# TtesseractT/Synthetic-Audio-Detection

Hardware: AMD Instinct MI355X
Metric: 4s@32kHz segments/sec end-to-end (mel+ResNet+ensemble), 1/2/4/8 MI355X (higher is better)
Workload: dtype bf16; 1 GPU; end-to-end inference: B int16 4 s segments resident in HBM -> mel front end -> ResNet-18@512x512 -> 6 binary heads -> merge (+RCCL all-gather of logits); heads=6, distinct_backbones=1, micro_batch=2048, parallelism=dp1, frontend_overlapped=True

## Files before the change

synthetic-audio-detection_amd/csrc/conv.hip:

```cpp
#include "common.hpp"
#include "kernels.hpp"
#include "igemm.hpp"

namespace sad {

template <int WM, int WN, int S>
constexpr int conv_smem_bytes() {
  constexpr int BM = 64 * WM, BN = 64 * WN;
  constexpr int main_b = S * (BM + BN) * 128;
  constexpr int epi_b = BM * (BN + 4) * 4;
  return main_b > epi_b ? main_b : epi_b;
}

template <typename T, int WM, int WN, int S>
__global__ __launch_bounds__(64 * WM * WN, 1) void conv_igemm_kernel(ConvArgs a) {
  static_assert(S == 2 || S == 3, "ring depth");
  constexpr int NW = WM * WN;
  constexpr int NT = 64 * NW;
  constexpr int BM = 64 * WM, BN = 64 * WN;
  constexpr int ES = sizeof(T);
  if (blockIdx.y > 0) {
    const int g = blockIdx.y;
    a.in = (const T*)a.in + g * a.in_gstride;
    a.wt = (const T*)a.wt + g * a.wt_gstride;
    a.bias = a.bias + g * a.bias_gstride;
    a.out = (T*)a.out + g * a.out_gstride;
  }
  constexpr int STAGE = (BM + BN) * 128;
  constexpr int QA = BM / 8 / NW;
  constexpr int QB = BN / 8 / NW;
  static_assert(QA * 8 * NW == BM && QB * 8 * NW == BN, "tile/wave mismatch");
  extern __shared__ __attribute__((aligned(16))) char smem[];

  const int tid = threadIdx.x, lane = tid & 63;
  const int wave = __builtin_amdgcn_readfirstlane(tid >> 6);
  const int wm = wave / WN, wn = wave % WN;
  const int n_tn = a.Cout / BN;
  const int wg = xcd_remap(blockIdx.x, gridDim.x);
  const int tn = wg % n_tn, tm = wg / n_tn;
  const int64_t m0 = (int64_t)tm * BM;
  const int n0 = tn * BN;
  const int HoWo = a.Ho * a.Wo;

  const __amdgpu_buffer_rsrc_t rin =
      __builtin_amdgcn_make_buffer_rsrc((void*)a.in, (short)0, (int)a.in_bytes, 0x00020000);
  const __amdgpu_buffer_rsrc_t rwt =
      __builtin_amdgcn_make_buffer_rsrc((void*)a.wt, (short)0, (int)a.wt_bytes, 0x00020000);
  const int pstride_b = (int)a.in_pstride * ES;

  const int lrow = lane >> 3;
  int aoff[QA], aiy[QA], aix[QA];
#pragma unroll
  for (int i = 0; i < QA; ++i) {
    const int r = 8 * (wave + NW * i) + lrow;
    const int c = (lane & 7) ^ ((r >> 1) & 7);
    const int64_t m = m0 + r;
    if (m < a.M) {
      const int b = (int)(m / HoWo);
      const int rem = (int)(m - (int64_t)b * HoWo);
      const int oy = rem / a.Wo, ox = rem - oy * a.Wo;
      aiy[i] = oy * a.stride - a.pad;
      aix[i] = ox * a.stride - a.pad;
      aoff[i] = ((b * a.H + aiy[i]) * a.W + aix[i]) * pstride_b + c * 16;
    } else {
      aiy[i] = -0x4000;
      aix[i] = -0x4000;
      aoff[i] = 0;
    }
  }
  const int ktot_b = a.KH * a.KW * a.Cin * ES;
  int boff[QB];
#pragma unroll
  for (int i = 0; i < QB; ++i) {
    const int r = 8 * (wave + NW * i) + lrow;
    const int c = (lane & 7) ^ (((r + BM) >> 1) & 7);
    boff[i] = (n0 + r) * ktot_b + c * 16;
  }
  const int cpt = a.Cin / (128 / ES);
  const int nk = a.KH * a.KW * cpt;

  const unsigned lds0 = (unsigned)(uintptr_t)(__attribute__((address_space(3))) char*)smem;
  auto issue = [&](int ks, int st) __attribute__((always_inline)) {
    const int tap = ks / cpt;
    const int ci0 = ks - tap * cpt;
    const int ky = tap / a.KW, kx = tap - ky * a.KW;
    const int toff = (ky * a.W + kx) * pstride_b + ci0 * 128;
    const unsigned sb = lds0 + st * STAGE;
#pragma unroll
    for (int i = 0; i < QA; ++i) {
      const int iy = aiy[i] + ky, ix = aix[i] + kx;
      const bool ok = ((unsigned)iy < (unsigned)a.H) && ((unsigned)ix < (unsigned)a.W);
      dma16(rin, ok ? aoff[i] + toff : 0x7FFFFFF0, sb + (wave + NW * i) * 1024);
    }
#pragma unroll
    for (int i = 0; i < QB; ++i) dma16(rwt, boff[i] + ks * 128, sb + BM * 128 + (wave + NW * i) * 1024);
  };

  f32x4 acc[4][4];
#pragma unroll
  for (int i = 0; i < 4; ++i)
#pragma unroll
    for (int j = 0; j < 4; ++j) acc[i][j] = f32x4{0.f, 0.f, 0.f, 0.f};

  const int fr = lane & 15, fg = lane >> 4;
  issue(0, 0);
  if (S == 3 && nk > 1) issue(1, 1);
  int st = 0;
  for (int ks = 0; ks < nk; ++ks) {
    if (S == 3 && ks + 1 < nk)
      asm volatile("s_waitcnt vmcnt(%0)" ::"n"(QA + QB) : "memory");
    else
      asm volatile("s_waitcnt vmcnt(0)" ::: "memory");
    __builtin_amdgcn_s_barrier();
    __builtin_amdgcn_sched_barrier(0);
    if (ks + S - 1 < nk) issue(ks + S - 1, S == 3 ? (st == 0 ? 2 : st - 1) : (st ^ 1));
    const char* base = smem + st * STAGE;
#pragma unroll
    for (int s = 0; s < 2; ++s) {
      uint4 af[4], bfr[4];
      const int c = fg + 4 * s;
#pragma unroll
      for (int i = 0; i < 4; ++i) {
        const int r = wm * 64 + i * 16 + fr;
        af[i] = *(const uint4*)(base + r * 128 + (swz(r, c) << 4));
      }
#pragma unroll
      for (int j = 0; j < 4; ++j) {
        const int r = BM + wn * 64 + j * 16 + fr;
        bfr[j] = *(const uint4*)(base + r * 128 + (swz(r, c) << 4));
      }
#pragma unroll
      for (int i = 0; i < 4; ++i)
#pragma unroll
        for (int j = 0; j < 4; ++j) mfma_chunk<T>(af[i], bfr[j], acc[i][j]);
    }
    st = st + 1 == S ? 0 : st + 1;
  }
  __syncthreads();

  float* ep = (float*)smem;
  constexpr int LDE = BN + 4;
#pragma unroll
  for (int i = 0; i < 4; ++i)
#pragma unroll
    for (int j = 0; j < 4; ++j)
#pragma unroll
      for (int r = 0; r < 4; ++r)
        ep[(wm * 64 + i * 16 + fg * 4 + r) * LDE + wn * 64 + j * 16 + fr] = acc[i][j][r];
  __syncthreads();
  constexpr int TPR = BN / 8;
  constexpr int RPP = NT / TPR;
  const int c8 = (tid % TPR) * 8;
  const float4 bias0 = *(const float4*)(a.bias + n0 + c8);
  const float4 bias1 = *(const float4*)(a.bias + n0 + c8 + 4);
  const T* __restrict__ res = (const T*)a.res;
  T* __restrict__ out = (T*)a.out;
  for (int row = tid / TPR; row < BM; row += RPP) {
    const int64_t m = m0 + row;
    if (m >= a.M) break;
    const float4 v0 = *(const float4*)(ep + row * LDE + c8);
    const float4 v1 = *(const float4*)(ep + row * LDE + c8 + 4);
    float v[8] = {v0.x + bias0.x, v0.y + bias0.y, v0.z + bias0.z, v0.w + bias0.w,
                  v1.x + bias1.x, v1.y + bias1.y, v1.z + bias1.z, v1.w + bias1.w};
    if (res) {
      const T* rp = res + m * a.res_pstride + n0 + c8;
      if constexpr (sizeof(T) == 2) {
        const uint4 q = *(const uint4*)rp;
        const u16* h = (const u16*)&q;
#pragma unroll
        for (int e = 0; e < 8; ++e) v[e] += bf2f(h[e]);
      } else {
        const float4 q0 = *(const float4*)rp, q1 = *(const float4*)(rp + 4);
        v[0] += q0.x; v[1] += q0.y; v[2] += q0.z; v[3] += q0.w;
        v[4] += q1.x; v[5] += q1.y; v[6] += q1.z; v[7] += q1.w;
      }
    }
    if (a.relu) {
#pragma unroll
      for (int e = 0; e < 8; ++e) v[e] = fmaxf(v[e], 0.f);
    }
    T* op = out + m * a.out_pstride + n0 + c8;
    if constexpr (sizeof(T) == 2) {
      uint4 q;
      u16* h = (u16*)&q;
#pragma unroll
      for (int e = 0; e < 8; ++e) h[e] = f2bf(v[e]);
      *(uint4*)op = q;
    } else {
      *(float4*)op = make_float4(v[0], v[1], v[2], v[3]);
      *(float4*)(op + 4) = make_float4(v[4], v[5], v[6], v[7]);
    }
  }
}

__device__ __forceinline__ float bilinear512(const float* __restrict__ map, int mh, int mw, float sh, float sw,
                                            int iy, int ix) {
  float fy = sh * (iy + 0.5f) - 0.5f;
  fy = fy < 0.f ? 0.f : fy;
  float fx = sw * (ix + 0.5f) - 0.5f;
  fx = fx < 0.f ? 0.f : fx;
  const int y0 = min((int)floorf(fy), mh - 1), x0 = min((int)floorf(fx), mw - 1);
  const int y1 = min(y0 + 1, mh - 1), x1 = min(x0 + 1, mw - 1);
  const float ly = fminf(fmaxf(fy - y0, 0.f), 1.f), lx = fminf(fmaxf(fx - x0, 0.f), 1.f);
  return (1.f - ly) * ((1.f - lx) * map[y0 * mw + x0] + lx * map[y0 * mw + x1]) +
         ly * ((1.f - lx) * map[y1 * mw + x0] + lx * map[y1 * mw + x1]);
}

constexpr int STEM_IMG_ROWS = 11;
constexpr int STEM_IMG_PITCH = 520;

template <typename T>
__global__ __launch_bounds__(256) void stem_kernel(StemArgs a) {
  constexpr int WPITCH = (64 * sizeof(T) + 16) / sizeof(T);
  __shared__ __attribute__((aligned(16))) float s_img[STEM_IMG_ROWS * STEM_IMG_PITCH];
  __shared__ __attribute__((aligned(16))) T s_w[64 * WPITCH];
  __shared__ __attribute__((aligned(16))) T s_pool[256 * 64];

  const int tid = threadIdx.x, lane = tid & 63, wave = tid >> 6;
  const int py = blockIdx.x;
  const int64_t b = blockIdx.y;
  const float* __restrict__ map = a.img ? nullptr : a.map + b * a.mh * a.mw;

  for (int i = tid; i < 64 * 64; i += 256) s_w[(i >> 6) * WPITCH + (i & 63)] = ((const T*)a.w)[i];
  const float sh = (float)a.mh / 512.f, sw = (float)a.mw / 512.f;
  for (int i = tid; i < STEM_IMG_ROWS * 517; i += 256) {
    const int tr = i / 517, tc = i - tr * 517;
    const int iy = 4 * py - 5 + tr, ix = tc - 3;
    float v = 0.f;
    if ((unsigned)iy < 512u && (unsigned)ix < 512u) {
      v = a.img ? a.img[(b * 512 + iy) * 512 + ix] : bilinear512(map, a.mh, a.mw, sh, sw, iy, ix);
      if constexpr (sizeof(T) == 2) v = bf2f(f2bf(v));
    }
    s_img[tr * STEM_IMG_PITCH + tc] = v;
  }
  __syncthreads();

  const int fr = lane & 15, fg = lane >> 4;
  int toff[16];
#pragma unroll
  for (int t = 0; t < 16; ++t) {
    int k;
    if constexpr (sizeof(T) == 2)
      k = 32 * (t >> 3) + 8 * fg + (t & 7);
    else
      k = 4 * t + fg;
    toff[t] = k < 49 ? (k / 7) * STEM_IMG_PITCH + (k % 7) : -1;
  }
  uint4 bw[4][2];
#pragma unroll
  for (int j = 0; j < 4; ++j) {
    const T* wr = s_w + (j * 16 + fr) * WPITCH;
    if constexpr (sizeof(T) == 2) {
      bw[j][0] = *(const uint4*)(wr + 8 * fg);
      bw[j][1] = *(const uint4*)(wr + 32 + 8 * fg);
    } else {
      bw[j][0] = *(const uint4*)(wr + 16 * fg);
      bw[j][1] = *(const uint4*)(wr + 16 * fg + 4);
    }
  }
  uint4 bw2[4][2];
  if constexpr (sizeof(T) == 4) {
#pragma unroll
    for (int j = 0; j < 4; ++j) {
      const T* wr = s_w + (j * 16 + fr) * WPITCH;
      bw2[j][0] = *(const uint4*)(wr + 16 * fg + 8);
      bw2[j][1] = *(const uint4*)(wr + 16 * fg + 12);
    }
  }

  f32x4 vmax[4][4];
#pragma unroll
  for (int i = 0; i < 4; ++i)
#pragma unroll
    for (int j = 0; j < 4; ++j) vmax[i][j] = f32x4{0.f, 0.f, 0.f, 0.f};

  for (int d = -1; d <= 1; ++d) {
    const int cr = 2 * py + d;
    if (cr < 0 || cr >= 256) continue;
    f32x4 acc[4][4];
#pragma unroll
    for (int i = 0; i < 4; ++i)
#pragma unroll
      for (int j = 0; j < 4; ++j) acc[i][j] = f32x4{0.f, 0.f, 0.f, 0.f};
#pragma unroll
    for (int i = 0; i < 4; ++i) {
      const int cx = wave * 64 + i * 16 + fr;
      const float* ib = s_img + (2 * d + 2) * STEM_IMG_PITCH + 2 * cx;
      float av[16];
#pragma unroll
      for (int t = 0; t < 16; ++t) av[t] = toff[t] >= 0 ? ib[toff[t]] : 0.f;
      if constexpr (sizeof(T) == 2) {
        uint4 a0, a1;
        u16* h0 = (u16*)&a0;
        u16* h1 = (u16*)&a1;
#pragma unroll
        for (int t = 0; t < 8; ++t) {
          h0[t] = f2bf(av[t]);
          h1[t] = f2bf(av[8 + t]);
        }
#pragma unroll
        for (int j = 0; j < 4; ++j) {
          mfma_chunk<u16>(a0, bw[j][0], acc[i][j]);
          mfma_chunk<u16>(a1, bw[j][1], acc[i][j]);
        }
      } else {
        const uint4 a0 = make_uint4(__float_as_uint(av[0]), __float_as_uint(av[1]), __float_as_uint(av[2]), __float_as_uint(av[3]));
        const uint4 a1 = make_uint4(__float_as_uint(av[4]), __float_as_uint(av[5]), __float_as_uint(av[6]), __float_as_uint(av[7]));
        const uint4 a2 = make_uint4(__float_as_uint(av[8]), __float_as_uint(av[9]), __float_as_uint(av[10]), __float_as_uint(av[11]));
        const uint4 a3 = make_uint4(__float_as_uint(av[12]), __float_as_uint(av[13]), __float_as_uint(av[14]), __float_as_uint(av[15]));
#pragma unroll
        for (int j = 0; j < 4; ++j) {
          mfma_chunk<float>(a0, bw[j][0], acc[i][j]);
          mfma_chunk<float>(a1, bw[j][1], acc[i][j]);
          mfma_chunk<float>(a2, bw2[j][0], acc[i][j]);
          mfma_chunk<float>(a3, bw2[j][1], acc[i][j]);
        }
      }
    }
#pragma unroll
    for (int j = 0; j < 4; ++j) {
      const float bj = a.bias[j * 16 + fr];
#pragma unroll
      for (int i = 0; i < 4; ++i)
#pragma unroll
        for (int r = 0; r < 4; ++r) {
          float v = fmaxf(acc[i][j][r] + bj, 0.f);
          if constexpr (sizeof(T) == 2) v = bf2f(f2bf(v));
          vmax[i][j][r] = fmaxf(vmax[i][j][r], v);
        }
    }
  }
#pragma unroll
  for (int i = 0; i < 4; ++i)
#pragma unroll
    for (int j = 0; j < 4; ++j)
#pragma unroll
      for (int r = 0; r < 4; ++r) {
        const int px = wave * 64 + i * 16 + fg * 4 + r;
        const float v = vmax[i][j][r];
        if constexpr (sizeof(T) == 2)
          s_pool[px * 64 + j * 16 + fr] = f2bf(v);
        else
          s_pool[px * 64 + j * 16 + fr] = v;
      }
  __syncthreads();
  T* __restrict__ out = (T*)a.out + ((b * 128 + py) * 128) * 64;
  for (int it = tid; it < 128 * 8; it += 256) {
    const int q = it >> 3, c0 = (it & 7) * 8;
    float m[8];
#pragma unroll
    for (int e = 0; e < 8; ++e) m[e] = 0.f;
    for (int px = 2 * q - 1; px <= 2 * q + 1; ++px) {
      if (px < 0 || px >= 256) continue;
#pragma unroll
      for (int e = 0; e < 8; ++e) {
        float v;
        if constexpr (sizeof(T) == 2)
          v = bf2f(s_pool[px * 64 + c0 + e]);
        else
          v = s_pool[px * 64 + c0 + e];
        m[e] = fmaxf(m[e], v);
      }
    }
    if constexpr (sizeof(T) == 2) {
      uint4 qv;
      u16* h = (u16*)&qv;
#pragma unroll
      for (int e = 0; e < 8; ++e) h[e] = f2bf(m[e]);
      *(uint4*)(out + q * 64 + c0) = qv;
    } else {
      *(float4*)(out + q * 64 + c0) = make_float4(m[0], m[1], m[2], m[3]);
      *(float4*)(out + q * 64 + c0 + 4) = make_float4(m[4], m[5], m[6], m[7]);
    }
  }
}

constexpr int STEM_P = 8;
constexpr int STEM_BAND_ROWS = 4 * STEM_P + 8;
constexpr int STEM_BPITCH = 544;
constexpr int STEM_HROWS = 12;
constexpr int STEM_UPITCH = 520;
constexpr int STEM_OPITCH = 128;
constexpr int STEM_WPITCH = 80;
__device__ __forceinline__ int stem_oswz(int q) { return ((q & 1) << 2) | (q & 2); }

typedef __bf16 stem_bf2 __attribute__((ext_vector_type(2)));
typedef float stem_f2 __attribute__((ext_vector_type(2)));
__device__ __forceinline__ uint32_t stem_pk(float lo, float hi) {
  return __builtin_bit_cast(uint32_t, __builtin_convertvector((stem_f2){lo, hi}, stem_bf2));
}
__device__ __forceinline__ uint32_t stem_relu2(uint32_t x) {
  uint32_t r;
  asm("v_pk_max_i16 %0, %1, 0" : "=v"(r) : "v"(x));
  return r;
}
template <int CTRL>
__device__ __forceinline__ float dppf(float v) {
  return __int_as_float(__builtin_amdgcn_update_dpp(0, __float_as_int(v), CTRL, 0xF, 0xF, true));
}

constexpr int STEM_OPITCH_X3 = 288;
constexpr int stem_u_build_floats() { return (STEM_HROWS + 1) * STEM_UPITCH + 4 * STEM_BAND_ROWS; }
template <bool X3>
constexpr int stem_u_floats() {
  return (X3 ? 128 * STEM_OPITCH_X3 / 4 : 128 * STEM_OPITCH / 4) + 256 > stem_u_build_floats()
             ? (X3 ? 128 * STEM_OPITCH_X3 / 4 : 128 * STEM_OPITCH / 4) + 256
             : stem_u_build_floats();
}

template <bool X3, bool TRAIN = false, bool X4 = false>
__global__ __launch_bounds__(256, X3 ? 1 : 2) void stem_bf16_kernel(StemArgs a) {
  static_assert(!(X3 && TRAIN), "the training stem is bf16");
  static_assert(!X4 || X3, "X4: the split stem's fourth product");
  constexpr int OPITCH = X3 ? STEM_OPITCH_X3 : STEM_OPITCH;
  __shared__ __attribute__((aligned(16))) u16 s_img[STEM_BAND_ROWS * STEM_BPITCH];
  __shared__ __attribute__((aligned(16))) u16 s_imgl[X3 ? STEM_BAND_ROWS * STEM_BPITCH : 8];
  __shared__ __attribute__((aligned(16))) u16 s_w[64 * STEM_WPITCH];
  __shared__ __attribute__((aligned(16))) u16 s_wl[X3 ? 64 * STEM_WPITCH : 8];
  __shared__ __attribute__((aligned(16))) float s_bias[64];
  __shared__ __attribute__((aligned(16))) float s_u[stem_u_floats<X3>()];
  char* s_out = (char*)s_u;
  float* s_edge = s_u + 128 * OPITCH / 4;

  const int tid = threadIdx.x, lane = tid & 63, wave = tid >> 6;
  const int py0 = blockIdx.x * STEM_P;
  const int64_t b = blockIdx.y;
  for (int i = tid; i < 64 * 8; i += 256) {
    const int co = i >> 3, c8 = (i & 7) * 8;
    uint4 wv = *(const uint4*)((const u16*)a.w + co * 64 + c8);
    if (TRAIN && a.bias[co] < 0.f) wv ^= make_uint4(0x80008000u, 0x80008000u, 0x80008000u, 0x80008000u);
    *(uint4*)(s_w + co * STEM_WPITCH + c8) = wv;
    if constexpr (X3)
      *(uint4*)(s_wl + co * STEM_WPITCH + c8) = *(const uint4*)((const u16*)a.w + 64 * 64 + co * 64 + c8);
  }
  auto put = [&](int i, float v) __attribute__((always_inline)) {
    const u16 h = f2bf(v);
    s_img[i] = h;
    if constexpr (X3) s_imgl[i] = f2bf(v - bf2f(h));
  };
  if (tid < 64) s_bias[tid] = TRAIN ? (a.bias[tid] < 0.f ? -1.f : 1.f) : a.bias[tid];
  constexpr int NBR = STEM_BAND_ROWS;
  if (TRAIN) {
    for (int i = tid; i < NBR * STEM_BPITCH; i += 256) {
      const int tr = i / STEM_BPITCH, tc = i - tr * STEM_BPITCH;
      const int iy = 4 * py0 - 5 + tr, ix = tc - 3;
      u16 v = 0;
      if ((unsigned)iy < 512u && (unsigned)ix < 512u) v = a.img16[(b * 512 + iy) * 512 + ix];
      s_img[i] = v;
    }
  } else if (a.img) {
    for (int i = tid; i < NBR * STEM_BPITCH; i += 256) {
      const int tr = i / STEM_BPITCH, tc = i - tr * STEM_BPITCH;
      const int iy = 4 * py0 - 5 + tr, ix = tc - 3;
      float v = 0.f;
      if ((unsigned)iy < 512u && (unsigned)ix < 512u) v = a.img[(b * 512 + iy) * 512 + ix];
      put(i, v);
    }
  } else {
    const float* __restrict__ map = a.map + b * a.mh * a.mw;
    const float sh = (float)a.mh / 512.f, sw = (float)a.mw / 512.f;
    auto src_row = [&](int iy, int& y0, int& y1, float& ly) {
      float fy = sh * (iy + 0.5f) - 0.5f;
      fy = fy < 0.f ? 0.f : fy;
      y0 = min((int)floorf(fy), a.mh - 1);
      y1 = min(y0 + 1, a.mh - 1);
      ly = fminf(fmaxf(fy - y0, 0.f), 1.f);
    };
    const int iy_lo = max(4 * py0 - 5, 0), iy_hi = min(4 * py0 - 5 + NBR - 1, 511);
    int ylo, yhi, t0, t1;
    float tl;
    src_row(iy_lo, ylo, t0, tl);
    src_row(iy_hi, t1, yhi, tl);
    const int nh = yhi - ylo + 1;
    if (nh <= STEM_HROWS) {
      constexpr int UP = STEM_UPITCH;
      float* s_zero = s_u + STEM_HROWS * UP;
      int4* s_rt = (int4*)(s_u + (STEM_HROWS + 1) * UP);
      int x0[2], x1[2];
      float lx[2];
#pragma unroll
      for (int c = 0; c < 2; ++c) {
        const int ix = tid + 256 * c;
        float fx = sw * (ix + 0.5f) - 0.5f;
        fx = fx < 0.f ? 0.f : fx;
        x0[c] = min((int)floorf(fx), a.mw - 1);
        x1[c] = min(x0[c] + 1, a.mw - 1);
        lx[c] = fminf(fmaxf(fx - x0[c], 0.f), 1.f);
      }
      float g0[STEM_HROWS][2], g1[STEM_HROWS][2];
#pragma unroll
      for (int r = 0; r < STEM_HROWS; ++r) {
        const float* mr = map + (ylo + min(r, nh - 1)) * a.mw;
#pragma unroll
        for (int c = 0; c < 2; ++c) {
          g0[r][c] = mr[x0[c]];
          g1[r][c] = mr[x1[c]];
        }
      }
#pragma unroll
      for (int r = 0; r < STEM_HROWS; ++r)
        if (r < nh) {
#pragma unroll
          for (int c = 0; c < 2; ++c) s_u[r * UP + 3 + tid + 256 * c] = (1.f - lx[c]) * g0[r][c] + lx[c] * g1[r][c];
        }
      if (tid < STEM_HROWS * 8) {
        const int r = tid >> 3, k = tid & 7;
        s_u[r * UP + (k < 3 ? k : 512 + k)] = 0.f;
      }
      for (int i = tid; i < UP; i += 256) s_zero[i] = 0.f;
      if (tid < NBR) {
        const int iy = 4 * py0 - 5 + tid;
        int4 rt = make_int4(STEM_HROWS * UP, STEM_HROWS * UP, __float_as_int(1.f), __float_as_int(0.f));
        if ((unsigned)iy < 512u) {
          int y0, y1;
          float ly;
          src_row(iy, y0, y1, ly);
          rt = make_int4((y0 - ylo) * UP, (y1 - ylo) * UP, __float_as_int(1.f - ly), __float_as_int(ly));
        }
        s_rt[tid] = rt;
      }
      __syncthreads();
      constexpr int QPR = (2 * 255 + 8 + 3) / 4;
      static_assert(4 * QPR <= UP && 4 * QPR <= STEM_BPITCH, "band quads");
#pragma unroll 2
      for (int it = tid; it < NBR * QPR; it += 256) {
        const int tr = it / QPR, q = it - tr * QPR;
        const int4 rt = s_rt[tr];
        const float w0 = __int_as_float(rt.z), w1 = __int_as_float(rt.w);
        const float4 u0 = *(const float4*)(s_u + rt.x + 4 * q);
        const float4 u1 = *(const float4*)(s_u + rt.y + 4 * q);
        const float v[4] = {w0 * u0.x + w1 * u1.x, w0 * u0.y + w1 * u1.y, w0 * u0.z + w1 * u1.z,
                            w0 * u0.w + w1 * u1.w};
        u16 h[4];
#pragma unroll
        for (int e = 0; e < 4; ++e) h[e] = f2bf(v[e]);
        const int o = tr * STEM_BPITCH + 4 * q;
        *(uint2*)(s_img + o) = make_uint2((uint32_t)h[0] | ((uint32_t)h[1] << 16), (uint32_t)h[2] | ((uint32_t)h[3] << 16));
        if constexpr (X3) {
          u16 l[4];
#pragma unroll
          for (int e = 0; e < 4; ++e) l[e] = f2bf(v[e] - bf2f(h[e]));
          *(uint2*)(s_imgl + o) =
              make_uint2((uint32_t)l[0] | ((uint32_t)l[1] << 16), (uint32_t)l[2] | ((uint32_t)l[3] << 16));
        }
      }
    } else {
      for (int i = tid; i < NBR * STEM_BPITCH; i += 256) {
        const int tr = i / STEM_BPITCH, tc = i - tr * STEM_BPITCH;
        const int iy = 4 * py0 - 5 + tr, ix = tc - 3;
        float v = 0.f;
        if ((unsigned)iy < 512u && (unsigned)ix < 512u) v = bilinear512(map, a.mh, a.mw, sh, sw, iy, ix);
        put(i, v);
      }
    }
  }
  __syncthreads();

  const int fr = lane & 15, fg = lane >> 4;

  auto conv_row = [&](int cr, f32x4 (&r)[4][4]) __attribute__((always_inline)) {
    const f32x4 init[4] = {};
    const int rb = 2 * (cr - 2 * py0) + 2;
    uint4 bw[4][2];
    uint4 bwl[X3 ? 4 : 1][2];
#pragma unroll
    for (int j = 0; j < 4; ++j)
#pragma unroll
      for (int s = 0; s < 2; ++s) {
        bw[j][s] = *(const uint4*)(s_w + (j * 16 + fr) * STEM_WPITCH + 32 * s + 8 * fg);
        if constexpr (X3) bwl[j][s] = *(const uint4*)(s_wl + (j * 16 + fr) * STEM_WPITCH + 32 * s + 8 * fg);
      }
#pragma unroll
    for (int i = 0; i < 4; ++i) {
      const int cx = wave * 64 + i * 16 + fr;
#pragma unroll
      for (int s = 0; s < 2; ++s) {
        const int o = (rb + 4 * s + fg) * STEM_BPITCH + 2 * cx;
        const u16* p = s_img + o;
        uint4 av;
        av.x = *(const uint32_t*)(p + 0);
        av.y = *(const uint32_t*)(p + 2);
        av.z = *(const uint32_t*)(p + 4);
        av.w = *(const uint32_t*)(p + 6);
#pragma unroll
        for (int j = 0; j < 4; ++j)
          r[i][j] = __builtin_amdgcn_mfma_f32_16x16x32_bf16(__builtin_bit_cast(bf16x8, av),
                                                            __builtin_bit_cast(bf16x8, bw[j][s]),
                                                            s == 0 ? init[j] : r[i][j], 0, 0, 0);
        if constexpr (X3) {
          const u16* pl = s_imgl + o;
          uint4 al;
          al.x = *(const uint32_t*)(pl + 0);
          al.y = *(const uint32_t*)(pl + 2);
          al.z = *(const uint32_t*)(pl + 4);
          al.w = *(const uint32_t*)(pl + 6);
#pragma unroll
          for (int j = 0; j < 4; ++j) mfma_chunk<u16>(av, bwl[j][s], r[i][j]);
#pragma unroll
          for (int j = 0; j < 4; ++j) mfma_chunk<u16>(al, bw[j][s], r[i][j]);
          if constexpr (X4) {
#pragma unroll
            for (int j = 0; j < 4; ++j) mfma_chunk<u16>(al, bwl[j][s], r[i][j]);
          }
        }
      }
    }
  };

  float st_s[4] = {0.f, 0.f, 0.f, 0.f}, st_q[4] = {0.f, 0.f, 0.f, 0.f};
  auto train_row = [&](const f32x4 (&r)[4][4]) __attribute__((always_inline)) {
#pragma unroll
    for (int i = 0; i < 4; ++i)
#pragma unroll
      for (int j = 0; j < 4; ++j)
#pragma unroll
        for (int e = 0; e < 4; ++e) {
          st_s[j] += r[i][j][e];
          st_q[j] += r[i][j][e] * r[i][j][e];
        }
  };
  f32x4 ca[4][4], cb[4][4], cur[4][4];
  if (py0 == 0) {
#pragma unroll
    for (int i = 0; i < 4; ++i)
#pragma unroll
      for (int j = 0; j < 4; ++j) ca[i][j] = f32x4{-INFINITY, -INFINITY, -INFINITY, -INFINITY};
  } else {
    conv_row(2 * py0 - 1, ca);
  }
  auto vmax = [](float x, float y) __attribute__((always_inline)) {
    if constexpr (TRAIN) return fmaxf(x, y);
    return __builtin_amdgcn_fmed3f(x, y, INFINITY);
  };
  auto pooled_row = [&](int pi, f32x4 (&carry)[4][4], f32x4 (&next)[4][4]) __attribute__((always_inline)) {
    __builtin_amdgcn_sched_barrier(0);
    const int py = py0 + pi;
    conv_row(2 * py, cur);
    if (TRAIN) train_row(cur);
#pragma unroll
    for (int i = 0; i < 4; ++i)
#pragma unroll
      for (int j = 0; j < 4; ++j) {
#pragma unroll
        for (int e = 0; e < 4; ++e) cur[i][j][e] = vmax(carry[i][j][e], cur[i][j][e]);
      }
    conv_row(2 * py + 1, next);
    if (TRAIN) train_row(next);
#pragma unroll
    for (int i = 0; i < 4; ++i)
#pragma unroll
      for (int j = 0; j < 4; ++j)
#pragma unroll
        for (int e = 0; e < 4; ++e) cur[i][j][e] = vmax(cur[i][j][e], next[i][j][e]);
    if (fg == 3) {
#pragma unroll
      for (int j = 0; j < 4; ++j) s_edge[wave * 64 + j * 16 + fr] = cur[3][j][3];
    }
    __syncthreads();
    float bias[4];
#pragma unroll
    for (int j = 0; j < 4; ++j) bias[j] = s_bias[j * 16 + fr];
    const bool even = (fr & 1) == 0;
#pragma unroll
    for (int i = 0; i < 4; ++i) {
#pragma unroll
      for (int j = 0; j < 4; ++j) {
        const f32x4 x = cur[i][j];
        const float send = fg == 3 ? (i > 0 ? cur[i - 1][j][3] : 0.f) : x[3];
        float left = __int_as_float(__builtin_amdgcn_ds_bpermute(((lane + 48) & 63) << 2, __float_as_int(send)));
        if (i == 0 && fg == 0) left = wave > 0 ? s_edge[(wave - 1) * 64 + j * 16 + fr] : -INFINITY;
        if constexpr (!X3 && !TRAIN) {
          const uint32_t pq = stem_relu2(stem_pk(fmaxf(fmaxf(left, x[0]), x[1]) + bias[j],
                                                 fmaxf(fmaxf(x[1], x[2]), x[3]) + bias[j]));
          const uint32_t pn = (uint32_t)__builtin_amdgcn_update_dpp(0, (int)pq, 0xB1, 0xF, 0xF, true);
          const uint32_t w = __builtin_amdgcn_perm(pn, pq, even ? 0x05040100u : 0x03020706u);
          const int q = wave * 32 + i * 8 + 2 * fg + (even ? 0 : 1);
          const int bo = (j * 16 + (fr & ~1)) * 2;
          *(uint32_t*)(s_out + q * OPITCH + ((((bo >> 4) ^ stem_oswz(q)) << 4) | (bo & 15))) = w;
          continue;
        }
        const float oa = TRAIN ? fmaxf(fmaxf(left, x[0]), x[1]) : fmaxf(fmaxf(fmaxf(left, x[0]), x[1]) + bias[j], 0.f);
        const float ob = TRAIN ? fmaxf(fmaxf(x[1], x[2]), x[3]) : fmaxf(fmaxf(fmaxf(x[1], x[2]), x[3]) + bias[j], 0.f);
        const float oa_next = dppf<0x101>(oa);
        const float ob_prev = dppf<0x111>(ob);
        const float v0 = even ? oa : ob_prev, v1 = even ? oa_next : ob;
        const int q = wave * 32 + i * 8 + 2 * fg + (even ? 0 : 1);
        const int c0 = j * 16 + (fr & ~1);
        const u16 h0 = f2bf(v0), h1 = f2bf(v1);
        if constexpr (X3) {
          const int pc = ((c0 >> 5) << 6) + (c0 & 31);
          *(uint32_t*)(s_out + q * OPITCH + pc * 2) = (uint32_t)h0 | ((uint32_t)h1 << 16);
          *(uint32_t*)(s_out + q * OPITCH + pc * 2 + 64) =
              (uint32_t)f2bf(v0 - bf2f(h0)) | ((uint32_t)f2bf(v1 - bf2f(h1)) << 16);
        } else {
          const int bo = c0 * 2;
          *(uint32_t*)(s_out + q * OPITCH + ((((bo >> 4) ^ stem_oswz(q)) << 4) | (bo & 15))) =
              (uint32_t)h0 | ((uint32_t)h1 << 16);
        }
      }
    }
    __syncthreads();
    constexpr int PXE = X3 ? 128 : 64;
    u16* __restrict__ out = (u16*)a.out + ((b * 128 + py) * 128) * PXE;
#pragma unroll
    for (int k = 0; k < PXE / 16; ++k) {
      const int idx = (k * 256 + tid) * 8;
      const int px = idx / PXE, c = (idx % PXE) / 8;
      *(uint4*)(out + idx) = *(const uint4*)(s_out + px * OPITCH + ((X3 ? c : c ^ stem_oswz(px)) << 4));
    }
    __syncthreads();
  };
  static_assert(STEM_P % 2 == 0, "pooled rows in pairs");
  if constexpr (TRAIN) {
    for (int pi = 0; pi < STEM_P; ++pi) {
      pooled_row(pi, ca, cb);
#pragma unroll
      for (int i = 0; i < 4; ++i)
#pragma unroll
        for (int j = 0; j < 4; ++j) ca[i][j] = cb[i][j];
    }
  } else {
    for (int pi = 0; pi < STEM_P; pi += 2) {
      pooled_row(pi, ca, cb);
      pooled_row(pi + 1, cb, ca);
    }
  }
  if constexpr (TRAIN) {
#pragma unroll
    for (int j = 0; j < 4; ++j) {
      st_s[j] += __shfl_xor(st_s[j], 16, 64);
      st_s[j] += __shfl_xor(st_s[j], 32, 64);
      st_q[j] += __shfl_xor(st_q[j], 16, 64);
      st_q[j] += __shfl_xor(st_q[j], 32, 64);
    }
    float* red = s_u;
    if (fg == 0) {
#pragma unroll
      for (int j = 0; j < 4; ++j) {
        red[wave * 128 + j * 16 + fr] = st_s[j];
        red[wave * 128 + 64 + j * 16 + fr] = st_q[j];
      }
    }
    __syncthreads();
    if (tid < 128) {
      const float v = (red[tid] + red[128 + tid]) + (red[256 + tid] + red[384 + tid]);
      a.part[((int64_t)blockIdx.y * gridDim.x + blockIdx.x) * 128 + tid] = tid < 64 ? v * s_bias[tid] : v;
    }
  }
}

constexpr int STEM3_PITCH = 520;
template <int OUT>
__global__ __launch_bounds__(128) void stem3_kernel(StemArgs a) {
  __shared__ float s_band[3 * STEM_IMG_ROWS * STEM3_PITCH];
  __shared__ __attribute__((aligned(16))) float s_w[64 * 148];
  const int tid = threadIdx.x;
  const int py = blockIdx.x;
  const int64_t b = blockIdx.y;
  for (int i = tid; i < 64 * 147; i += 128) s_w[(i / 147) * 148 + i % 147] = a.w3[i];
  const float* img = a.img3 + b * 3 * 512 * 512;
  for (int i = tid; i < 3 * STEM_IMG_ROWS * STEM3_PITCH; i += 128) {
    const int c = i / (STEM_IMG_ROWS * STEM3_PITCH), r = i % (STEM_IMG_ROWS * STEM3_PITCH);
    const int tr = r / STEM3_PITCH, tc = r % STEM3_PITCH;
    const int iy = 4 * py - 5 + tr, ix = tc - 5;
    s_band[i] = ((unsigned)iy < 512u && (unsigned)ix < 512u) ? img[((int64_t)c * 512 + iy) * 512 + ix] : 0.f;
  }
  __syncthreads();
  const int px = tid;
  float pooled[64];
#pragma unroll
  for (int j = 0; j < 64; ++j) pooled[j] = 0.f;
  for (int g = 0; g < 4; ++g) {
    float best[16];
#pragma unroll
    for (int j = 0; j < 16; ++j) best[j] = 0.f;
    for (int dy = -1; dy <= 1; ++dy) {
      const int cy = 2 * py + dy;
      if (cy < 0 || cy >= 256) continue;
      for (int dx = -1; dx <= 1; ++dx) {
        const int cx = 2 * px + dx;
        if (cx < 0 || cx >= 256) continue;
        float acc[16];
#pragma unroll
        for (int j = 0; j < 16; ++j) acc[j] = a.bias[g * 16 + j];
        for (int c = 0; c < 3; ++c)
          for (int ky = 0; ky < 7; ++ky) {
            const float* br = s_band + (c * STEM_IMG_ROWS + (2 * cy - 3 + ky) - (4 * py - 5)) * STEM3_PITCH + 2 * cx + 2;
            for (int kx = 0; kx < 7; ++kx) {
              const float v = br[kx];
              const float* wr = s_w + (g * 16) * 148 + c * 49 + ky * 7 + kx;
#pragma unroll
              for (int j = 0; j < 16; ++j) acc[j] = fmaf(v, wr[j * 148], acc[j]);
            }
          }
#pragma unroll
        for (int j = 0; j < 16; ++j) best[j] = fmaxf(best[j], acc[j]);
      }
    }
#pragma unroll
    for (int j = 0; j < 16; ++j) pooled[g * 16 + j] = best[j];
  }
  const int64_t pix = (b * 128 + py) * 128 + px;
  if constexpr (OUT == 0) {
    float* o = (float*)a.out + pix * 64;
#pragma unroll
    for (int j = 0; j < 64; j += 4) *(float4*)(o + j) = make_float4(pooled[j], pooled[j + 1], pooled[j + 2], pooled[j + 3]);
  } else if constexpr (OUT == 1) {
    u16* o = (u16*)a.out + pix * 64;
#pragma unroll
    for (int j = 0; j < 64; ++j) o[j] = f2bf(pooled[j]);
  } else {
    u16* o = (u16*)a.out + pix * 128;
#pragma unroll
    for (int j = 0; j < 64; ++j) {
      const u16 h = f2bf(pooled[j]);
      o[(j >> 5) * 64 + (j & 31)] = h;
      o[(j >> 5) * 64 + 32 + (j & 31)] = f2bf(pooled[j] - bf2f(h));
    }
  }
}

template <typename T, bool X3 = false>
__global__ __launch_bounds__(256) void avgpool_kernel(const T* __restrict__ in, int hw, int c,
                                                      float* __restrict__ out) {
  __shared__ float part[4][64];
  const int64_t b = blockIdx.x;
  const int ch = blockIdx.y * 64 + (threadIdx.x & 63), g = threadIdx.x >> 6;
  const int pc = X3 ? ((ch >> 5) << 6) + (ch & 31) : ch;
  const int ps = X3 ? 2 * c : c;
  const T* p = in + b * hw * ps + pc;
  float s = 0.f;
  for (int i = g; i < hw; i += 4) {
    if constexpr (X3)
      s += bf2f(p[(int64_t)i * ps]) + bf2f(p[(int64_t)i * ps + 32]);
    else if constexpr (sizeof(T) == 2)
      s += bf2f(p[(int64_t)i * c]);
    else
      s += p[(int64_t)i * c];
  }
  part[g][threadIdx.x & 63] = s;
  __syncthreads();
  if (g == 0) {
    const int t = threadIdx.x;
    out[b * c + ch] = ((part[0][t] + part[1][t]) + (part[2][t] + part[3][t])) / (float)hw;
  }
}

template <typename T, int WM, int WN, int S>
static int launch_conv_t(const ConvArgs& a, hipStream_t s) {
  constexpr int BM = 64 * WM, BN = 64 * WN;
  constexpr int smem = conv_smem_bytes<WM, WN, S>();
  static bool attr = false;
  if (!attr) {
    (void)hipFuncSetAttribute((const void*)conv_igemm_kernel<T, WM, WN, S>,
                              hipFuncAttributeMaxDynamicSharedMemorySize, smem);
    attr = true;
  }
  SAD_REQUIRE(a.Cout % BN == 0, "Cout must be a multiple of the tile width");
  const int64_t tiles_m = (a.M + BM - 1) / BM;
  const int64_t nwg = tiles_m * (a.Cout / BN);
  SAD_REQUIRE(nwg < (1ll << 31), "grid too large");
  SAD_REQUIRE(a.groups <= 1 || !a.res, "grouped conv: no residual");
  hipLaunchKernelGGL((conv_igemm_kernel<T, WM, WN, S>), dim3((unsigned)nwg, (unsigned)std::max(a.groups, 1)),
                     dim3(64 * WM * WN), smem, s, a);
  SAD_CHECK_HIP(hipGetLastError());
  return SAD_OK;
}

template <typename T>
static int launch_conv_v(const ConvArgs& a, int v, hipStream_t s) {
  switch (v) {
    case 1: return launch_conv_t<T, 4, 1, 3>(a, s);
    case 2: return launch_conv_t<T, 4, 1, 2>(a, s);
    case 3: return launch_conv_t<T, 4, 2, 3>(a, s);
    case 4: return launch_conv_t<T, 2, 2, 3>(a, s);
    case 5: return launch_conv_t<T, 2, 2, 2>(a, s);
    case 6: return launch_conv_t<T, 8, 1, 2>(a, s);
    case 7: return launch_conv_t<T, 2, 1, 3>(a, s);
    case 8: return launch_conv_t<T, 4, 2, 2>(a, s);
  }
  set_error("unknown conv variant");
  return SAD_ERR_ARG;
}

int default_conv_variant(const ConvArgs& a) { return a.Cout % 128 == 0 ? 5 : 2; }

int launch_conv(const ConvArgs& a_in, int dtype, hipStream_t s, int variant) {
  const int EPC = dtype == SAD_BF16 ? 8 : 4;
  const int ES = dtype == SAD_BF16 ? 2 : 4;
  ConvArgs a = a_in;
  a.in_bytes = (((int64_t)a.N * a.H * a.W - 1) * a.in_pstride + a.Cin) * ES;
  a.wt_bytes = (int64_t)a.Cout * a.KH * a.KW * a.Cin * ES;
  SAD_REQUIRE(a.in_bytes < (1ll << 31) - 64 && a.wt_bytes < (1ll << 31),
              "conv operand exceeds the 2 GiB buffer range (lower the micro-batch)");
  SAD_REQUIRE(a.Cin % (8 * EPC) == 0, "Cin must be a multiple of the K-step");
  SAD_REQUIRE(a.Cout % 64 == 0, "Cout must be a multiple of 64");
  SAD_REQUIRE(a.in_pstride % EPC == 0 && a.out_pstride % 8 == 0, "pixel strides must keep 16-B alignment");
  if (a.M == 0) return SAD_OK;
  const int v = variant > 0 ? variant : default_conv_variant(a);
  return dtype == SAD_BF16 ? launch_conv_v<u16>(a, v, s) : launch_conv_v<float>(a, v, s);
}

int launch_stem(const StemArgs& a, int dtype, hipStream_t s) {
  SAD_REQUIRE(a.B <= 65535, "stem: B > 65535");
  if (a.B == 0) return SAD_OK;
  if (a.img3) {
    SAD_REQUIRE(a.w3 && a.bias, "distinct-channel stem: weights");
    if (dtype == SAD_F32)
      hipLaunchKernelGGL(stem3_kernel<0>, dim3(128, (unsigned)a.B), dim3(128), 0, s, a);
    else if (dtype == SAD_BF16)
      hipLaunchKernelGGL(stem3_kernel<1>, dim3(128, (unsigned)a.B), dim3(128), 0, s, a);
    else
      hipLaunchKernelGGL(stem3_kernel<2>, dim3(128, (unsigned)a.B), dim3(128), 0, s, a);
    SAD_CHECK_HIP(hipGetLastError());
    return SAD_OK;
  }
  if (dtype == SAD_BF16)
    hipLaunchKernelGGL(stem_bf16_kernel<false>, dim3(128 / STEM_P, (unsigned)a.B), dim3(256), 0, s, a);
  else if (dtype == SAD_BF16X3 && a.x4)
    hipLaunchKernelGGL((stem_bf16_kernel<true, false, true>), dim3(128 / STEM_P, (unsigned)a.B), dim3(256), 0, s, a);
  else if (dtype == SAD_BF16X3)
    hipLaunchKernelGGL(stem_bf16_kernel<true>, dim3(128 / STEM_P, (unsigned)a.B), dim3(256), 0, s, a);
  else
    hipLaunchKernelGGL(stem_kernel<float>, dim3(128, (unsigned)a.B), dim3(256), 0, s, a);
  SAD_CHECK_HIP(hipGetLastError());
  return SAD_OK;
}

int launch_stem_train(const StemArgs& a, hipStream_t s) {
  SAD_REQUIRE(a.B <= 65535, "stem: B > 65535");
  SAD_REQUIRE(a.img16 && a.w && a.bias && a.out && a.part, "training stem: null argument");
  if (a.B == 0) return SAD_OK;
  hipLaunchKernelGGL((stem_bf16_kernel<false, true>), dim3(128 / STEM_P, (unsigned)a.B), dim3(256), 0, s, a);
  SAD_CHECK_HIP(hipGetLastError());
  return SAD_OK;
}

int launch_avgpool(const void* in, int64_t B, int hw, int c, float* out, int dtype, hipStream_t s) {
  if (B == 0) return SAD_OK;
  if (dtype == SAD_BF16X3)
    hipLaunchKernelGGL((avgpool_kernel<u16, true>), dim3((unsigned)B, c / 64), dim3(256), 0, s, (const u16*)in, hw, c,
                       out);
  else if (dtype == SAD_BF16)
    hipLaunchKernelGGL(avgpool_kernel<u16>, dim3((unsigned)B, c / 64), dim3(256), 0, s, (const u16*)in, hw, c, out);
  else
    hipLaunchKernelGGL(avgpool_kernel<float>, dim3((unsigned)B, c / 64), dim3(256), 0, s, (const float*)in, hw, c, out);
  SAD_CHECK_HIP(hipGetLastError());
  return SAD_OK;
}

}
```

Measured before the change: 63270 segments/s.

## Fuse stem max-pool into MFMA register epilogue with rolling row reuse

Adds an HP variant of the bf16 inference stem that computes the 3x3/stride-2 max-pool directly from MFMA accumulators in registers. Column order is permuted so adjacent outputs share lanes, and vertical pooling reuses the previous conv row through ping-pong register sets. Only boundary columns cross lanes via ds_bpermute and a small LDS edge buffer. This drops the LDS staging of conv rows before pooling, and the band pitch shrinks to 520, at the cost of extra registers, a __syncthreads per pooled row and an env-gated code path that is on by default.

After: 63710 segments/s, median of 6. Within noise of the previous version (+0.7%).

```diff
diff --git a/synthetic-audio-detection_amd/csrc/conv.hip b/synthetic-audio-detection_amd/csrc/conv.hip
--- a/synthetic-audio-detection_amd/csrc/conv.hip
+++ b/synthetic-audio-detection_amd/csrc/conv.hip
@@ -378,11 +378,16 @@
 constexpr int STEM_P = 8;
 constexpr int STEM_BAND_ROWS = 4 * STEM_P + 8;
 constexpr int STEM_BPITCH = 544;
+constexpr int STEM_BPITCH_HP = 520;
 constexpr int STEM_HROWS = 12;
 constexpr int STEM_UPITCH = 520;
 constexpr int STEM_OPITCH = 128;
 constexpr int STEM_WPITCH = 80;
 __device__ __forceinline__ int stem_oswz(int q) { return ((q & 1) << 2) | (q & 2); }
+__device__ __forceinline__ constexpr int stem_hp_col(int w, int i, int m) {
+  return 64 * w + 32 * (i >> 1) + 8 * (m >> 2) + 4 * (i & 1) + (m & 3);
+}
+__device__ __forceinline__ constexpr int stem_hp_q(int w, int h, int fg, int k) { return 32 * w + 16 * h + 4 * fg + k; }
 
 typedef __bf16 stem_bf2 __attribute__((ext_vector_type(2)));
 typedef float stem_f2 __attribute__((ext_vector_type(2)));
@@ -408,13 +413,15 @@
              : stem_u_build_floats();
 }
 
-template <bool X3, bool TRAIN = false, bool X4 = false>
+template <bool X3, bool TRAIN = false, bool X4 = false, bool HP = false>
 __global__ __launch_bounds__(256, X3 ? 1 : 2) void stem_bf16_kernel(StemArgs a) {
   static_assert(!(X3 && TRAIN), "the training stem is bf16");
   static_assert(!X4 || X3, "X4: the split stem's fourth product");
+  static_assert(!HP || (!X3 && !TRAIN), "HP: the bf16 inference stem's pool");
   constexpr int OPITCH = X3 ? STEM_OPITCH_X3 : STEM_OPITCH;
-  __shared__ __attribute__((aligned(16))) u16 s_img[STEM_BAND_ROWS * STEM_BPITCH];
-  __shared__ __attribute__((aligned(16))) u16 s_imgl[X3 ? STEM_BAND_ROWS * STEM_BPITCH : 8];
+  constexpr int BPITCH = HP ? STEM_BPITCH_HP : STEM_BPITCH;
+  __shared__ __attribute__((aligned(16))) u16 s_img[STEM_BAND_ROWS * BPITCH];
+  __shared__ __attribute__((aligned(16))) u16 s_imgl[X3 ? STEM_BAND_ROWS * BPITCH : 8];
   __shared__ __attribute__((aligned(16))) u16 s_w[64 * STEM_WPITCH];
   __shared__ __attribute__((aligned(16))) u16 s_wl[X3 ? 64 * STEM_WPITCH : 8];
   __shared__ __attribute__((aligned(16))) float s_bias[64];
@@ -441,16 +448,16 @@
   if (tid < 64) s_bias[tid] = TRAIN ? (a.bias[tid] < 0.f ? -1.f : 1.f) : a.bias[tid];
   constexpr int NBR = STEM_BAND_ROWS;
   if (TRAIN) {
-    for (int i = tid; i < NBR * STEM_BPITCH; i += 256) {
-      const int tr = i / STEM_BPITCH, tc = i - tr * STEM_BPITCH;
+    for (int i = tid; i < NBR * BPITCH; i += 256) {
+      const int tr = i / BPITCH, tc = i - tr * BPITCH;
       const int iy = 4 * py0 - 5 + tr, ix = tc - 3;
       u16 v = 0;
       if ((unsigned)iy < 512u && (unsigned)ix < 512u) v = a.img16[(b * 512 + iy) * 512 + ix];
       s_img[i] = v;
     }
   } else if (a.img) {
-    for (int i = tid; i < NBR * STEM_BPITCH; i += 256) {
-      const int tr = i / STEM_BPITCH, tc = i - tr * STEM_BPITCH;
+    for (int i = tid; i < NBR * BPITCH; i += 256) {
+      const int tr = i / BPITCH, tc = i - tr * BPITCH;
       const int iy = 4 * py0 - 5 + tr, ix = tc - 3;
       float v = 0.f;
       if ((unsigned)iy < 512u && (unsigned)ix < 512u) v = a.img[(b * 512 + iy) * 512 + ix];
@@ -521,7 +528,7 @@
       }
       __syncthreads();
       constexpr int QPR = (2 * 255 + 8 + 3) / 4;
-      static_assert(4 * QPR <= UP && 4 * QPR <= STEM_BPITCH, "band quads");
+      static_assert(4 * QPR <= UP && 4 * QPR <= BPITCH, "band quads");
 #pragma unroll 2
       for (int it = tid; it < NBR * QPR; it += 256) {
         const int tr = it / QPR, q = it - tr * QPR;
@@ -534,7 +541,7 @@
         u16 h[4];
 #pragma unroll
         for (int e = 0; e < 4; ++e) h[e] = f2bf(v[e]);
-        const int o = tr * STEM_BPITCH + 4 * q;
+        const int o = tr * BPITCH + 4 * q;
         *(uint2*)(s_img + o) = make_uint2((uint32_t)h[0] | ((uint32_t)h[1] << 16), (uint32_t)h[2] | ((uint32_t)h[3] << 16));
         if constexpr (X3) {
           u16 l[4];
@@ -545,8 +552,8 @@
         }
       }
     } else {
-      for (int i = tid; i < NBR * STEM_BPITCH; i += 256) {
-        const int tr = i / STEM_BPITCH, tc = i - tr * STEM_BPITCH;
+      for (int i = tid; i < NBR * BPITCH; i += 256) {
+        const int tr = i / BPITCH, tc = i - tr * BPITCH;
         const int iy = 4 * py0 - 5 + tr, ix = tc - 3;
         float v = 0.f;
         if ((unsigned)iy < 512u && (unsigned)ix < 512u) v = bilinear512(map, a.mh, a.mw, sh, sw, iy, ix);
@@ -557,6 +564,114 @@
   __syncthreads();
 
   const int fr = lane & 15, fg = lane >> 4;
+
+  if constexpr (HP) {
+    auto max2 = [](float x, float y) __attribute__((always_inline)) { return __builtin_amdgcn_fmed3f(x, y, INFINITY); };
+    auto max3 = [&](float x, float y, float z) __attribute__((always_inline)) { return max2(max2(x, y), z); };
+    uint4 bw[4][2];
+#pragma unroll
+    for (int j = 0; j < 4; ++j)
+#pragma unroll
+      for (int s = 0; s < 2; ++s) bw[j][s] = *(const uint4*)(s_w + (4 * fr + j) * STEM_WPITCH + 32 * s + 8 * fg);
+    const u16* const abase = s_img + fg * BPITCH + 2 * stem_hp_col(wave, 0, fr);
+    auto hrow = [&](int cr, f32x4 (&P)[2][4], float (&E)[2][4]) __attribute__((always_inline)) {
+      const f32x4 init[4] = {};
+      int o0 = (2 * (cr - 2 * py0) + 2) * BPITCH, o1 = o0 + 4 * BPITCH;
+      asm volatile("" : "+v"(o0), "+v"(o1));
+      const u16* const prow[2] = {abase + o0, abase + o1};
+      f32x4 r[4][4];
+#pragma unroll
+      for (int i = 0; i < 4; ++i)
+#pragma unroll
+        for (int s = 0; s < 2; ++s) {
+          const u16* p = prow[s] + 2 * stem_hp_col(0, i, 0);
+          uint4 av;
+          av.x = *(const uint32_t*)(p + 0);
+          av.y = *(const uint32_t*)(p + 2);
+          av.z = *(const uint32_t*)(p + 4);
+          av.w = *(const uint32_t*)(p + 6);
+#pragma unroll
+          for (int j = 0; j < 4; ++j)
+            r[i][j] = __builtin_amdgcn_mfma_f32_16x16x32_bf16(__builtin_bit_cast(bf16x8, av),
+                                                              __builtin_bit_cast(bf16x8, bw[j][s]),
+                                                              s == 0 ? init[j] : r[i][j], 0, 0, 0);
+        }
+#pragma unroll
+      for (int h = 0; h < 2; ++h)
+#pragma unroll
+        for (int j = 0; j < 4; ++j) {
+          const f32x4 lo = r[2 * h][j], hi = r[2 * h + 1][j];
+          P[h][j][0] = max2(lo[0], lo[1]);
+          P[h][j][1] = max3(lo[1], lo[2], lo[3]);
+          P[h][j][2] = max3(lo[3], hi[0], hi[1]);
+          P[h][j][3] = max3(hi[1], hi[2], hi[3]);
+          E[h][j] = hi[3];
+        }
+    };
+    f32x4 pa[2][4], pb[2][4];
+    float ea[2][4], eb[2][4];
+    if (py0 == 0) {
+#pragma unroll
+      for (int h = 0; h < 2; ++h)
+#pragma unroll
+        for (int j = 0; j < 4; ++j) {
+          pa[h][j] = f32x4{-INFINITY, -INFINITY, -INFINITY, -INFINITY};
+          ea[h][j] = -INFINITY;
+        }
+    } else {
+      hrow(2 * py0 - 1, pa, ea);
+    }
+    auto pooled_row = [&](int pi, f32x4 (&cP)[2][4], float (&cE)[2][4], f32x4 (&nP)[2][4], float (&nE)[2][4])
+                          __attribute__((always_inline)) {
+      __builtin_amdgcn_sched_barrier(0);
+      const int py = py0 + pi;
+      f32x4 P[2][4];
+      float E[2][4];
+      hrow(2 * py, P, E);
+      __builtin_amdgcn_sched_barrier(0);
+      hrow(2 * py + 1, nP, nE);
+#pragma unroll
+      for (int h = 0; h < 2; ++h)
+#pragma unroll
+        for (int j = 0; j < 4; ++j) {
+#pragma unroll
+          for (int k = 0; k < 4; ++k) P[h][j][k] = max3(cP[h][j][k], P[h][j][k], nP[h][j][k]);
+          E[h][j] = max3(cE[h][j], E[h][j], nE[h][j]);
+        }
+      float* edge = s_u + (pi & 1) * 256;
+      if (fg == 3) {
+#pragma unroll
+        for (int j = 0; j < 4; ++j) edge[wave * 64 + j * 16 + fr] = E[1][j];
+      }
+      __syncthreads();
+#pragma unroll
+      for (int j = 0; j < 4; ++j) {
+        const float r0 = __int_as_float(__builtin_amdgcn_ds_bpermute(((lane + 48) & 63) << 2, __float_as_int(E[0][j])));
+        const float r1 = __int_as_float(__builtin_amdgcn_ds_bpermute(((lane + 48) & 63) << 2, __float_as_int(E[1][j])));
+        float l0 = r0, l1 = r1;
+        if (fg == 0) {
+          l1 = r0;
+          l0 = wave > 0 ? edge[(wave - 1) * 64 + j * 16 + fr] : -INFINITY;
+        }
+        P[0][j][0] = max2(P[0][j][0], l0);
+        P[1][j][0] = max2(P[1][j][0], l1);
+      }
+      const float4 bias = *(const float4*)(s_bias + 4 * fr);
+      u16* __restrict__ out = (u16*)a.out + ((b * 128 + py) * 128) * 64 + 4 * fr;
+#pragma unroll
+      for (int h = 0; h < 2; ++h)
+#pragma unroll
+        for (int k = 0; k < 4; ++k)
+          *(uint2*)(out + stem_hp_q(wave, h, fg, k) * 64) =
+              make_uint2(stem_relu2(stem_pk(P[h][0][k] + bias.x, P[h][1][k] + bias.y)),
+                         stem_relu2(stem_pk(P[h][2][k] + bias.z, P[h][3][k] + bias.w)));
+    };
+    for (int pi = 0; pi < STEM_P; pi += 2) {
+      pooled_row(pi, pa, ea, pb, eb);
+      pooled_row(pi + 1, pb, eb, pa, ea);
+    }
+    return;
+  }
 
   auto conv_row = [&](int cr, f32x4 (&r)[4][4]) __attribute__((always_inline)) {
     const f32x4 init[4] = {};
@@ -575,7 +690,7 @@
       const int cx = wave * 64 + i * 16 + fr;
 #pragma unroll
       for (int s = 0; s < 2; ++s) {
-        const int o = (rb + 4 * s + fg) * STEM_BPITCH + 2 * cx;
+        const int o = (rb + 4 * s + fg) * BPITCH + 2 * cx;
         const u16* p = s_img + o;
         uint4 av;
         av.x = *(const uint32_t*)(p + 0);
@@ -901,6 +1016,14 @@
   return dtype == SAD_BF16 ? launch_conv_v<u16>(a, v, s) : launch_conv_v<float>(a, v, s);
 }
 
+static bool stem_pool_hp() {
+  static const bool v = [] {
+    const char* e = getenv("SAD_STEM_POOL");
+    return e ? atoi(e) != 0 : true;
+  }();
+  return v;
+}
+
 int launch_stem(const StemArgs& a, int dtype, hipStream_t s) {
   SAD_REQUIRE(a.B <= 65535, "stem: B > 65535");
   if (a.B == 0) return SAD_OK;
@@ -915,7 +1038,10 @@
     SAD_CHECK_HIP(hipGetLastError());
     return SAD_OK;
   }
-  if (dtype == SAD_BF16)
+  if (dtype == SAD_BF16 && stem_pool_hp())
+    hipLaunchKernelGGL((stem_bf16_kernel<false, false, false, true>), dim3(128 / STEM_P, (unsigned)a.B), dim3(256), 0, s,
+                       a);
+  else if (dtype == SAD_BF16)
     hipLaunchKernelGGL(stem_bf16_kernel<false>, dim3(128 / STEM_P, (unsigned)a.B), dim3(256), 0, s, a);
   else if (dtype == SAD_BF16X3 && a.x4)
     hipLaunchKernelGGL((stem_bf16_kernel<true, false, true>), dim3(128 / STEM_P, (unsigned)a.B), dim3(256), 0, s, a);
```
